# 17LiQi/MultimodalSignal

Hardware: AMD Instinct MI355X
Metric: train windows/sec (higher is better)
Workload: dtype f32; 1 GPU; CnnGruAttentionModel full train step (fwd+CE+bwd+Adam, dropout 0.5, BN batch stats), B=8192 windows/GPU x (6 ch, 3840 samples = 60 s @ 64 Hz), random-init weights; BASELINE.json configs[4] shape, the per-step work of configs[1]; batch_per_gpu=8192, channels=6, samples=3840, classes=2, parallelism=replica x1

## Files before the change

### multimodalsignal_amd/csrc/frontend.hip

```cpp
#include "msig_dev.h"

template <int CT, bool EO_ONLY = false>
__global__ __launch_bounds__(256) void gate_kernel(const float* __restrict__ x, const float* __restrict__ W1,
                                                   const float* __restrict__ W2, float* __restrict__ mean_out,
                                                   float* __restrict__ pre_out, float* __restrict__ s_out,
                                                   float* __restrict__ eo_out, int C, int T, int Cr, const FoldCtx fc) {
  FOLD_BEGIN; FS(x); FS(W1); FS(W2); FS(mean_out); FS(pre_out); FS(s_out); FS(eo_out);
  __shared__ float red[4][MSIG_MAX_C];
  __shared__ float red_eo[4][2 * MSIG_MAX_C];
  __shared__ float mean_s[MSIG_MAX_C];
  __shared__ float hid_s[MSIG_MAX_C / 4];
  const int b = blockIdx.x, tid = threadIdx.x, lane = tid & 63, w = tid >> 6;
  const float* xb = x + (size_t)b * C * T;
  if (CT > 0 && (T & 3) == 0) {
    constexpr int CN = CT > 0 ? CT : 1;
    float acc[CN], ev[CN], od[CN];
#pragma unroll
    for (int c = 0; c < CN; ++c) acc[c] = ev[c] = od[c] = 0.f;
    const int T4 = T / 4;
    constexpr int U = CN <= 4 ? 4 : 2;
    for (int i0 = tid; i0 < T4; i0 += 256 * U) {
      float4 q[U][CN];
#pragma unroll
      for (int u = 0; u < U; ++u) {
        const int i = i0 + 256 * u < T4 ? i0 + 256 * u : i0;
#pragma unroll
        for (int c = 0; c < CN; ++c) q[u][c] = ((const float4*)xb)[(size_t)c * T4 + i];
      }
#pragma unroll
      for (int u = 0; u < U; ++u)
        if (i0 + 256 * u < T4) {
#pragma unroll
          for (int c = 0; c < CN; ++c) {
            if (!EO_ONLY) acc[c] += (q[u][c].x + q[u][c].y) + (q[u][c].z + q[u][c].w);
            ev[c] += q[u][c].x + q[u][c].z; od[c] += q[u][c].y + q[u][c].w;
          }
        }
    }
#pragma unroll
    for (int c = 0; c < CN; ++c) {
      if (!EO_ONLY) {
        const float a = wave_sum(acc[c]);
        if (lane == 0) red[w][c] = a;
      }
      if (eo_out) {
        const float e = wave_sum(ev[c]), o = wave_sum(od[c]);
        if (lane == 0) { red_eo[w][2 * c] = e; red_eo[w][2 * c + 1] = o; }
      }
    }
  } else
  for (int c = 0; c < C; ++c) {
    const float* xc = xb + (size_t)c * T;
    float acc = 0.f, ev = 0.f, od = 0.f;
    if ((T & 3) == 0) {
      const float4* x4 = (const float4*)xc;
      for (int i = tid; i < T / 4; i += 256) {
        const float4 q = x4[i];
        if (!EO_ONLY) acc += (q.x + q.y) + (q.z + q.w);
        ev += q.x + q.z; od += q.y + q.w;
      }
    } else {
      for (int i = tid; i < T; i += 256) { const float v = xc[i]; if (!EO_ONLY) acc += v; if (i & 1) od += v; else ev += v; }
    }
    if (!EO_ONLY) {
      acc = wave_sum(acc);
      if (lane == 0) red[w][c] = acc;
    }
    if (eo_out) {
      ev = wave_sum(ev); od = wave_sum(od);
      if (lane == 0) { red_eo[w][2 * c] = ev; red_eo[w][2 * c + 1] = od; }
    }
  }
  __syncthreads();
  if (EO_ONLY) {
    if (tid < 2 * C) eo_out[(size_t)b * 2 * C + tid] = (red_eo[0][tid] + red_eo[1][tid]) + (red_eo[2][tid] + red_eo[3][tid]);
    return;
  }
  if (tid < C) {
    const float m = (red[0][tid] + red[1][tid] + red[2][tid] + red[3][tid]) / (float)T;
    mean_s[tid] = m;
    mean_out[(size_t)b * C + tid] = m;
  }
  if (eo_out && tid < 2 * C) eo_out[(size_t)b * 2 * C + tid] = (red_eo[0][tid] + red_eo[1][tid]) + (red_eo[2][tid] + red_eo[3][tid]);
  __syncthreads();
  if (tid < Cr) {
    float a = 0.f;
    for (int c = 0; c < C; ++c) a += W1[tid * C + c] * mean_s[c];
    pre_out[(size_t)b * Cr + tid] = a;
    hid_s[tid] = a > 0.f ? a : 0.f;
  }
  __syncthreads();
  if (tid < C) {
    float a = 0.f;
    for (int j = 0; j < Cr; ++j) a += W2[tid * Cr + j] * hid_s[j];
    s_out[(size_t)b * C + tid] = sigmoidf_fast(a);
  }
}

__global__ __launch_bounds__(256) void gate_scale_kernel(const float* __restrict__ x, const float* __restrict__ s, float* __restrict__ out,
                                                         int T, int64_t n_rows) {
  for (int64_t row = blockIdx.x; row < n_rows; row += gridDim.x) {
    const float sc = s[row];
    const float* xr = x + row * T;
    float* o = out + row * T;
    if ((T & 3) == 0 && (((uintptr_t)xr | (uintptr_t)o) & 15) == 0) {
      for (int i = threadIdx.x; i < T / 4; i += 256) {
        const float4 q = ((const float4*)xr)[i];
        ((float4*)o)[i] = make_float4(q.x * sc, q.y * sc, q.z * sc, q.w * sc);
      }
    } else {
      for (int i = threadIdx.x; i < T; i += 256) o[i] = xr[i] * sc;
    }
  }
}
int launch_channel_attention(const float* x, const float* W1, const float* W2, int B, int C, int T, float* out, float* s, float* scratch,
                             hipStream_t st) {
  const int Cr = C / 4;
  const FoldCtx fc = single_fold(nullptr);
  gate_kernel<0><<<dim3(B, 1, 1), 256, 0, st>>>(x, W1, W2, scratch, scratch + (size_t)B * C, s, nullptr, C, T, Cr, fc);
  MSIG_LAUNCH_CHECK();
  const int64_t rows = (int64_t)B * C;
  gate_scale_kernel<<<dim3((unsigned)(rows < 4096 ? rows : 4096)), 256, 0, st>>>(x, s, out, T, rows);
  MSIG_LAUNCH_CHECK();
  return 0;
}

#define C1_CHUNK 256
#define C1_XW (2 * C1_CHUNK + 8)
#define C1_XP (C1_XW / 2 + 4)
#define C1_MAXKM 28

template <bool DEINT>
__device__ __forceinline__ void stage_x_chunk(float* xs, const float* __restrict__ xb, int C, int T, int t0, int tid, int xstride = C1_XW) {
  const int g_base = 2 * t0 - 4;
  if ((T & 3) == 0) {
    for (int i = tid; i < C * (C1_XW / 4); i += 256) {
      const int c = i / (C1_XW / 4), i4 = i - c * (C1_XW / 4), g0 = g_base + 4 * i4;
      const int gc = g0 < 0 ? 0 : (g0 > T - 4 ? T - 4 : g0);
      float4 q = *(const float4*)(xb + (size_t)c * T + gc);
      if (g0 < 0 || g0 > T - 4) q = make_float4(0.f, 0.f, 0.f, 0.f);
      if (DEINT) {
        *(float2*)&xs[(2 * c) * C1_XP + 2 * i4] = make_float2(q.x, q.z);
        *(float2*)&xs[(2 * c + 1) * C1_XP + 2 * i4] = make_float2(q.y, q.w);
      } else {
        *(float4*)&xs[c * xstride + 4 * i4] = q;
      }
    }
  } else {
    for (int i = tid; i < C * C1_XW; i += 256) {
      const int c = i / C1_XW, j = i - c * C1_XW, g = g_base + j;
      const int gc = g < 0 ? 0 : (g > T - 1 ? T - 1 : g);
      float v = xb[(size_t)c * T + gc];
      if (g < 0 || g > T - 1 - (msig_negctl_length == 1 && t0 > 0 ? 1 : 0)) v = 0.f;
      if (DEINT) xs[(2 * c + (j & 1)) * C1_XP + (j >> 1)] = v; else xs[c * xstride + j] = v;
    }
  }
}

template <int CT, bool GATED = true>
__global__ __launch_bounds__(256) void conv1_fwd_kernel(const float* __restrict__ x, const float* __restrict__ w1,
                                                        const float* __restrict__ gate_s, float* __restrict__ y1,
                                                        float* __restrict__ part, int B, int Crt, int T, int L1,
                                                        int want_stats, const FoldCtx fc) {
  FOLD_BEGIN; FS(x); FS(w1); FS(gate_s); FS(y1); FS(part);
  extern __shared__ __attribute__((aligned(16))) float smem[];
  const int C = CT > 0 ? CT : Crt;
  const int K = C * 7, KM = (K + 3) / 4;
  constexpr int KMC = CT > 0 ? (CT * 7 + 3) / 4 : C1_MAXKM;
  float* xs = smem;
  float* ws = smem + 2 * C * C1_XP;
  const int tid = threadIdx.x, lane = tid & 63, w = tid >> 6, li = lane & 15, lq = lane >> 4;
  int xo[KMC];
#pragma unroll
  for (int m = 0; m < KMC; ++m) {
    const int k = 4 * m + lq, kc = k < K ? k : 0, c = kc / 7, kk = kc - 7 * c;
    xo[m] = (2 * c + ((kk + 1) & 1)) * C1_XP + ((kk + 1) >> 1);
  }
  const int nchunk = (L1 + C1_CHUNK - 1) / C1_CHUNK;
  const int nitems = B * nchunk;
  f32x4 ssum = {0.f, 0.f, 0.f, 0.f}, ssq = {0.f, 0.f, 0.f, 0.f};
  f32x4 dsum = {0.f, 0.f, 0.f, 0.f}, dsq = {0.f, 0.f, 0.f, 0.f}, piv = {0.f, 0.f, 0.f, 0.f};
  int nacc = 0;
  constexpr bool PIPE = CT > 0;
  constexpr int NX4 = PIPE ? (CT * (C1_XW / 4) + 255) / 256 : 1;
  constexpr int NWS = PIPE ? (4 * KMC * 16 + 255) / 256 : 1;
  const bool pipe = PIPE && (T & 3) == 0;
  float4 xr[NX4];
  float wfix[NWS], gr[NWS];
  if (GATED && pipe) {
#pragma unroll
    for (int j = 0; j < NWS; ++j) {
      const int i = tid + 256 * j, k = i >> 4, o = i & 15;
      wfix[j] = (i < 4 * KM * 16 && k < K) ? w1[o * K + k] : 0.f;
    }
  }
  auto prefetch = [&](int item) {
    const int b = item / nchunk, t0 = (item - b * nchunk) * C1_CHUNK, g_base = 2 * t0 - 4;
    const float* xb = x + (size_t)b * C * T;
#pragma unroll
    for (int j = 0; j < NX4; ++j) {
      const int i = tid + 256 * j, ic = i < C * (C1_XW / 4) ? i : 0;
      const int c = ic / (C1_XW / 4), i4 = ic - c * (C1_XW / 4), g0 = g_base + 4 * i4;
      const int gc = g0 < 0 ? 0 : (g0 > T - 4 ? T - 4 : g0);
      xr[j] = *(const float4*)(xb + (size_t)c * T + gc);
    }
    if (GATED) {
#pragma unroll
      for (int j = 0; j < NWS; ++j) {
        const int i = tid + 256 * j, k = i >> 4, kc = (i < 4 * KM * 16 && k < K) ? k : 0;
        gr[j] = gate_s[(size_t)b * C + kc / 7];
      }
    }
  };
  float wa[KMC];
  if (!GATED) {
#pragma unroll
    for (int m = 0; m < KMC; ++m) {
      const int k = 4 * m + lq;
      wa[m] = ((CT > 0 || m < KM) && k < K) ? w1[li * K + k] : 0.f;
    }
  }
  if (pipe && (int)blockIdx.x < nitems) prefetch(blockIdx.x);
  for (int item = blockIdx.x; item < nitems; item += gridDim.x) {
    const int b = item / nchunk, t0 = (item - b * nchunk) * C1_CHUNK;
    __syncthreads();
    if (pipe) {
      const int g_base = 2 * t0 - 4;
#pragma unroll
      for (int j = 0; j < NX4; ++j) {
        const int i = tid + 256 * j;
        if (i < C * (C1_XW / 4)) {
          const int c = i / (C1_XW / 4), i4 = i - c * (C1_XW / 4), g0 = g_base + 4 * i4;
          float4 q = xr[j];
          if (g0 < 0 || g0 > T - 4) q = make_float4(0.f, 0.f, 0.f, 0.f);
          *(float2*)&xs[(2 * c) * C1_XP + 2 * i4] = make_float2(q.x, q.z);
          *(float2*)&xs[(2 * c + 1) * C1_XP + 2 * i4] = make_float2(q.y, q.w);
        }
      }
      if (GATED) {
#pragma unroll
        for (int j = 0; j < NWS; ++j) {
          const int i = tid + 256 * j;
          if (i < 4 * KM * 16) ws[i] = wfix[j] * gr[j];
        }
      }
    } else {
      stage_x_chunk<true>(xs, x + (size_t)b * C * T, C, T, t0, tid);
      if (GATED) {
        for (int i = tid; i < 4 * KM * 16; i += 256) {
          const int k = i >> 4, o = i & 15, kc = k < K ? k : 0;
          const float v = w1[o * K + kc] * gate_s[(size_t)b * C + kc / 7];
          ws[i] = (k < K || (msig_negctl_range == 1 && CT == 0)) ? v : 0.f;
        }
      }
    }
    __syncthreads();
    if (pipe && item + (int)gridDim.x < nitems) prefetch(item + gridDim.x);
    if (GATED) {
#pragma unroll
      for (int m = 0; m < KMC; ++m) wa[m] = (CT > 0 || m < KM) ? ws[(4 * m + lq) * 16 + li] : 0.f;
    }
#pragma unroll
    for (int pbi = 0; pbi < 4; ++pbi) {
      const int pl = (w * 4 + pbi) * 16 + li;
      f32x4 acc0 = {0.f, 0.f, 0.f, 0.f}, acc1 = {0.f, 0.f, 0.f, 0.f};
#pragma unroll
      for (int m = 0; m < KMC; m += 2) {
        if (CT > 0 || m < KM) acc0 = mfma16(wa[m], xs[xo[m] + pl], acc0);
        if (m + 1 < KMC && (CT > 0 || m + 1 < KM)) acc1 = mfma16(wa[m + 1], xs[xo[m + 1] + pl], acc1);
      }
      const f32x4 acc = acc0 + acc1;
      const int t = t0 + pl;
      if (t < L1) {
        *(float4*)(y1 + ((size_t)b * L1 + t) * 16 + lq * 4) = make_float4(acc[0], acc[1], acc[2], acc[3]);
#pragma unroll
        for (int e = 0; e < 4; ++e) { ssum[e] += acc[e]; ssq[e] += acc[e] * acc[e]; }
        if (nacc == 0) piv = acc;
        ++nacc;
#pragma unroll
        for (int e = 0; e < 4; ++e) { const float dv = acc[e] - piv[e]; dsum[e] += dv; dsq[e] += dv * dv; }
      }
    }
  }
  if (want_stats) {
    __syncthreads();
    float* red = smem;
#pragma unroll
    for (int e = 0; e < 4; ++e) {
      float s1 = ssum[e], s2 = ssq[e];
#pragma unroll
      for (int o = 8; o > 0; o >>= 1) { s1 += __shfl_xor(s1, o, 64); s2 += __shfl_xor(s2, o, 64); }
      if (li == 0) { red[w * 32 + lq * 4 + e] = s1; red[w * 32 + 16 + lq * 4 + e] = s2; }
    }
    __syncthreads();
    if (tid < 32) part[(size_t)blockIdx.x * 32 + tid] = red[tid] + red[32 + tid] + red[64 + tid] + red[96 + tid];
    double* redd = (double*)(smem + 4 * 32);
#pragma unroll
    for (int e = 0; e < 4; ++e) {
      double s1, s2;
      bn_unshift(nacc, piv[e], dsum[e], dsq[e], s1, s2);
#pragma unroll
      for (int o = 8; o > 0; o >>= 1) { s1 += __shfl_xor(s1, o, 64); s2 += __shfl_xor(s2, o, 64); }
      if (li == 0) { redd[w * 32 + lq * 4 + e] = s1; redd[w * 32 + 16 + lq * 4 + e] = s2; }
    }
    __syncthreads();
    if (tid < 32) bn_shifted_part(part, 16)[(size_t)blockIdx.x * 32 + tid] = (redd[tid] + redd[32 + tid]) + (redd[64 + tid] + redd[96 + tid]);
  }
}

#define C2_CHUNK 128
#define C2_ROWS (2 * C2_CHUNK + 3)
#define C2_PS 20
#define PC_YROWS (2 * C2_ROWS + 1)
__device__ __forceinline__ int first_argmax3(float l, float c, float r);
__global__ __launch_bounds__(256, 2) void pool1_conv2_fwd_kernel(const float* __restrict__ y1, const float* __restrict__ stat1,
                                                                 float* __restrict__ p1, uint8_t* __restrict__ code1,
                                                                 const float* __restrict__ w2, float* __restrict__ y2,
                                                                 float* __restrict__ part, int B, int L1, int P1, int L2,
                                                                 int want_stats, const FoldCtx fc) {
  FOLD_BEGIN; FS(y1); FS(stat1); FS(p1); FS(code1); FS(w2); FS(y2); FS(part);
  __shared__ __attribute__((aligned(16))) float zs[PC_YROWS * C2_PS];
  __shared__ __attribute__((aligned(16))) float ps[C2_ROWS * C2_PS];
  __shared__ float red[4 * 64];
  const int tid = threadIdx.x, lane = tid & 63, w = tid >> 6, li = lane & 15, lq = lane >> 4;
  float A[2][20];
#pragma unroll
  for (int ob = 0; ob < 2; ++ob)
#pragma unroll
    for (int m = 0; m < 20; ++m) A[ob][m] = w2[((ob * 16 + li) * 16 + lq * 4 + (m & 3)) * 5 + (m >> 2)];
  const int nchunk = (L2 + C2_CHUNK - 1) / C2_CHUNK;
  const int nitems = B * nchunk;
  f32x4 ssum[2] = {{0.f, 0.f, 0.f, 0.f}, {0.f, 0.f, 0.f, 0.f}}, ssq[2] = {{0.f, 0.f, 0.f, 0.f}, {0.f, 0.f, 0.f, 0.f}};
  f32x4 dsum[2] = {{0.f, 0.f, 0.f, 0.f}, {0.f, 0.f, 0.f, 0.f}}, dsq[2] = {{0.f, 0.f, 0.f, 0.f}, {0.f, 0.f, 0.f, 0.f}};
  f32x4 piv[2] = {{0.f, 0.f, 0.f, 0.f}, {0.f, 0.f, 0.f, 0.f}};
  int nacc = 0;
  const float NINF = -__builtin_huge_valf();
  const int c4s = tid & 3;
  const float4 sc4 = *(const float4*)(stat1 + 2 * 16 + c4s * 4), sh4 = *(const float4*)(stat1 + 3 * 16 + c4s * 4);
  const float scv[4] = {sc4.x, sc4.y, sc4.z, sc4.w}, shv[4] = {sh4.x, sh4.y, sh4.z, sh4.w};
  constexpr int NY4 = (PC_YROWS * 4 + 255) / 256, NP4 = (C2_ROWS * 4 + 255) / 256;
  float4 yr[NY4];
  auto prefetch = [&](int item) {
    const int b = item / nchunk, t0 = (item - b * nchunk) * C2_CHUNK, ty0 = 4 * t0 - 5;
#pragma unroll
    for (int j = 0; j < NY4; ++j) {
      const int i = tid + 256 * j, row = i >> 2, ty = ty0 + row;
      const int tc = ty < 0 ? 0 : (ty > L1 - 1 ? L1 - 1 : ty);
      yr[j] = *(const float4*)(y1 + ((size_t)b * L1 + tc) * 16 + c4s * 4);
    }
  };
  if ((int)blockIdx.x < nitems) prefetch(blockIdx.x);
  for (int item = blockIdx.x; item < nitems; item += gridDim.x) {
    const int b = item / nchunk, t0 = (item - b * nchunk) * C2_CHUNK;
    const int base = 2 * t0 - 2, ty0 = 4 * t0 - 5;
    __syncthreads();
#pragma unroll
    for (int j = 0; j < NY4; ++j) {
      const int i = tid + 256 * j, row = i >> 2, ty = ty0 + row;
      if (i < PC_YROWS * 4) {
        const bool ok = ty >= 0 && ty < L1;
        const float qv[4] = {yr[j].x, yr[j].y, yr[j].z, yr[j].w};
        float z[4];
#pragma unroll
        for (int e = 0; e < 4; ++e) z[e] = ok ? qv[e] * scv[e] + shv[e] : NINF;
        *(float4*)&zs[row * C2_PS + c4s * 4] = make_float4(z[0], z[1], z[2], z[3]);
      }
    }
    __syncthreads();
    if (item + (int)gridDim.x < nitems) prefetch(item + gridDim.x);
#pragma unroll
    for (int j = 0; j < NP4; ++j) {
      const int i = tid + 256 * j, row = i >> 2, pp = base + row;
      if (i < C2_ROWS * 4) {
        float best[4] = {0.f, 0.f, 0.f, 0.f};
        if (pp >= 0 && pp < P1) {
          const float4 l4 = *(const float4*)&zs[(2 * row) * C2_PS + c4s * 4], m4 = *(const float4*)&zs[(2 * row + 1) * C2_PS + c4s * 4],
                       r4 = *(const float4*)&zs[(2 * row + 2) * C2_PS + c4s * 4];
          const float zl[4] = {l4.x, l4.y, l4.z, l4.w}, zc[4] = {m4.x, m4.y, m4.z, m4.w}, zr[4] = {r4.x, r4.y, r4.z, r4.w};
          unsigned cd = 0;
#pragma unroll
          for (int e = 0; e < 4; ++e) {
            const int win = first_argmax3(zl[e], zc[e], zr[e]);
            const float m = win == 0 ? zl[e] : (win == 1 ? zc[e] : zr[e]);
            best[e] = fmaxf(m, 0.f);
            cd |= (unsigned)(m > 0.f ? win : 3) << (2 * e);
          }
          if (row >= 2 && row < 2 + 2 * C2_CHUNK) {
            *(float4*)(p1 + ((size_t)b * P1 + pp) * 16 + c4s * 4) = make_float4(best[0], best[1], best[2], best[3]);
            if (code1) code1[((size_t)b * P1 + pp) * 4 + c4s] = (uint8_t)cd;
          }
        }
        *(float4*)&ps[row * C2_PS + c4s * 4] = make_float4(best[0], best[1], best[2], best[3]);
      }
    }
    __syncthreads();
#pragma unroll
    for (int pbi = 0; pbi < 2; ++pbi) {
      const int pl = (w * 2 + pbi) * 16 + li;
      f32x4 acc0 = {0.f, 0.f, 0.f, 0.f}, acc1 = {0.f, 0.f, 0.f, 0.f};
#pragma unroll
      for (int kk = 0; kk < 5; ++kk) {
        const float4 q = *(const float4*)&ps[(2 * pl + kk) * C2_PS + lq * 4];
        acc0 = mfma16(A[0][4 * kk + 0], q.x, acc0); acc1 = mfma16(A[1][4 * kk + 0], q.x, acc1);
        acc0 = mfma16(A[0][4 * kk + 1], q.y, acc0); acc1 = mfma16(A[1][4 * kk + 1], q.y, acc1);
        acc0 = mfma16(A[0][4 * kk + 2], q.z, acc0); acc1 = mfma16(A[1][4 * kk + 2], q.z, acc1);
        acc0 = mfma16(A[0][4 * kk + 3], q.w, acc0); acc1 = mfma16(A[1][4 * kk + 3], q.w, acc1);
      }
      const int t = t0 + pl;
      if (t < L2) {
        float* dst = y2 + ((size_t)b * L2 + t) * 32 + lq * 4;
        *(float4*)dst = make_float4(acc0[0], acc0[1], acc0[2], acc0[3]);
        *(float4*)(dst + 16) = make_float4(acc1[0], acc1[1], acc1[2], acc1[3]);
#pragma unroll
        for (int e = 0; e < 4; ++e) {
          ssum[0][e] += acc0[e]; ssq[0][e] += acc0[e] * acc0[e];
          ssum[1][e] += acc1[e]; ssq[1][e] += acc1[e] * acc1[e];
        }
        if (nacc == 0) { piv[0] = acc0; piv[1] = acc1; }
        ++nacc;
#pragma unroll
        for (int e = 0; e < 4; ++e) {
          const float d0 = acc0[e] - piv[0][e], d1 = acc1[e] - piv[1][e];
          dsum[0][e] += d0; dsq[0][e] += d0 * d0;
          dsum[1][e] += d1; dsq[1][e] += d1 * d1;
        }
      }
    }
  }
  if (want_stats) {
#pragma unroll
    for (int ob = 0; ob < 2; ++ob)
#pragma unroll
      for (int e = 0; e < 4; ++e) {
        float s1 = ssum[ob][e], s2 = ssq[ob][e];
#pragma unroll
        for (int o = 8; o > 0; o >>= 1) { s1 += __shfl_xor(s1, o, 64); s2 += __shfl_xor(s2, o, 64); }
        if (li == 0) { red[w * 64 + ob * 16 + lq * 4 + e] = s1; red[w * 64 + 32 + ob * 16 + lq * 4 + e] = s2; }
      }
    __syncthreads();
    if (tid < 64) part[(size_t)blockIdx.x * 64 + tid] = red[tid] + red[64 + tid] + red[128 + tid] + red[192 + tid];
    double* redd = (double*)zs;
#pragma unroll
    for (int ob = 0; ob < 2; ++ob)
#pragma unroll
      for (int e = 0; e < 4; ++e) {
        double s1, s2;
        bn_unshift(nacc, piv[ob][e], dsum[ob][e], dsq[ob][e], s1, s2);
#pragma unroll
        for (int o = 8; o > 0; o >>= 1) { s1 += __shfl_xor(s1, o, 64); s2 += __shfl_xor(s2, o, 64); }
        if (li == 0) { redd[w * 64 + ob * 16 + lq * 4 + e] = s1; redd[w * 64 + 32 + ob * 16 + lq * 4 + e] = s2; }
      }
    __syncthreads();
    if (tid < 64) bn_shifted_part(part, 32)[(size_t)blockIdx.x * 64 + tid] = (redd[tid] + redd[64 + tid]) + (redd[128 + tid] + redd[192 + tid]);
  }
}


__global__ __launch_bounds__(FIN_THREADS) void bn_finalize_kernel(const float* __restrict__ part, int nrows, int CH, double count,
                                                          const float* __restrict__ gamma, const float* __restrict__ beta,
                                                          float* __restrict__ run_mean, float* __restrict__ run_var,
                                                          int64_t* __restrict__ nbt, float momentum, float eps,
                                                          int training, float* __restrict__ stat, const FoldCtx fc) {
  FOLD_BEGIN; FS(part); FS(gamma); FS(beta); FS(run_mean); FS(run_var); FS(nbt); FS(stat);
  __shared__ double red[FIN_THREADS];
  const int tid = threadIdx.x;
  if (training) {
    double s1, s2;
    const bool shifted = bn_batch_sums(part, nrows, CH, count, red, s1, s2);
    if (tid < CH) {
      const double mean = s1 / count;
      double var = s2 / count - mean * mean;
      if (var < 0.0) var = 0.0;
      const float invstd = (float)(msig_negctl_input == 2 ? 1.0 / (sqrt(var) + (double)eps) : 1.0 / sqrt(var + (double)eps));
      const float sc = (msig_negctl_regime == 3 ? fabsf(gamma[tid]) : gamma[tid]) * invstd;
      stat[tid] = (float)mean;
      stat[CH + tid] = invstd;
      stat[2 * CH + tid] = sc;
      stat[3 * CH + tid] = beta[tid] - (float)mean * sc;
      stat[4 * CH + tid] = shifted ? (float)((mean - (double)(float)mean) * (double)invstd) : 0.f;
      const double unbiased = count > 1.0 ? var * count / (count - 1.0) : var;
      float new_mean, new_var;
      bn_running_update(momentum, (float)mean, (float)unbiased, run_mean[tid], run_var[tid], new_mean, new_var);
      run_mean[tid] = new_mean;
      run_var[tid] = new_var;
    }
    if (tid == 0) nbt[0] += 1;
  } else if (tid < CH) {
    const float invstd = 1.0f / sqrtf(run_var[tid] + eps);
    const float sc = (msig_negctl_regime == 3 ? fabsf(gamma[tid]) : gamma[tid]) * invstd;
    stat[tid] = run_mean[tid];
    stat[CH + tid] = invstd;
    stat[2 * CH + tid] = sc;
    stat[3 * CH + tid] = beta[tid] - run_mean[tid] * sc;
    stat[4 * CH + tid] = 0.f;
  }
}

__device__ __forceinline__ int first_argmax3(float l, float c, float r) {
  int a = 0; float m = l;
  if (c > m) { a = 1; m = c; }
  if (r > m) { a = 2; }
  return a;
}

template <int CH>
__global__ __launch_bounds__(256) void bn_relu_pool_kernel(const float* __restrict__ y, const float* __restrict__ stat,
                                                           float* __restrict__ p, uint8_t* __restrict__ code, int B, int L, int P,
                                                           const FoldCtx fc) {
  FOLD_BEGIN; FS(y); FS(stat); FS(p); FS(code);
  constexpr int C4 = CH / 4;
  const int64_t total = (int64_t)B * P * C4;
  const float NINF = -__builtin_huge_valf();
  for (int64_t i = (int64_t)blockIdx.x * 256 + threadIdx.x; i < total; i += (int64_t)gridDim.x * 256) {
    const int c4 = (int)(i % C4);
    const int64_t bp = i / C4;
    const int pp = (int)(bp % P), b = (int)(bp / P);
    const float4 sc = *(const float4*)(stat + 2 * CH + c4 * 4), sh = *(const float4*)(stat + 3 * CH + c4 * 4);
    const float scv[4] = {sc.x, sc.y, sc.z, sc.w}, shv[4] = {sh.x, sh.y, sh.z, sh.w};
    float z[3][4];
#pragma unroll
    for (int j = 0; j < 3; ++j) {
      const int t = 2 * pp - 1 + j;
      const bool ok = t >= 0 && t < L;
      const float4 q = *(const float4*)(y + ((size_t)b * L + (ok ? t : 2 * pp)) * CH + c4 * 4);
      const float qv[4] = {q.x, q.y, q.z, q.w};
#pragma unroll
      for (int e = 0; e < 4; ++e) z[j][e] = ok ? qv[e] * scv[e] + shv[e] : NINF;
    }
    float best[4];
    unsigned cd = 0;
#pragma unroll
    for (int e = 0; e < 4; ++e) {
      const int win = first_argmax3(z[0][e], z[1][e], z[2][e]);
      const float m = win == 0 ? z[0][e] : (win == 1 ? z[1][e] : z[2][e]);
      best[e] = fmaxf(m, 0.f);
      cd |= (unsigned)(m > 0.f ? win : 3) << (2 * e);
    }
    *(float4*)(p + ((size_t)b * P + pp) * CH + c4 * 4) = make_float4(best[0], best[1], best[2], best[3]);
    if (code) code[((size_t)b * P + pp) * C4 + c4] = (uint8_t)cd;
  }
}

struct RoutedRaw { float4 g0, g1; unsigned c0, c1; };
template <int CH>
__device__ __forceinline__ RoutedRaw routed_load(const float* __restrict__ dp, const uint8_t* __restrict__ code, int b, int t, int P, int c4) {
  constexpr int C4 = CH / 4;
  const int ph = t >> 1, ph1 = (ph + 1 < P) ? ph + 1 : ph;
  RoutedRaw r;
  r.g0 = *(const float4*)(dp + ((size_t)b * P + ph) * CH + c4 * 4);
  r.g1 = *(const float4*)(dp + ((size_t)b * P + ph1) * CH + c4 * 4);
  r.c0 = code[((size_t)b * P + ph) * C4 + c4];
  r.c1 = code[((size_t)b * P + ph1) * C4 + c4];
  return r;
}
__device__ __forceinline__ float4 routed_dz(const RoutedRaw& r, int t, int P) {
  const bool odd = t & 1, has1 = odd && ((t >> 1) + 1 < P);
  const unsigned want0 = odd ? 2u : 1u;
  const float g0[4] = {r.g0.x, r.g0.y, r.g0.z, r.g0.w}, g1[4] = {r.g1.x, r.g1.y, r.g1.z, r.g1.w};
  float o[4];
#pragma unroll
  for (int e = 0; e < 4; ++e) {
    o[e] = (((r.c0 >> (2 * e)) & 3u) == want0) ? g0[e] : 0.f;
    if (has1 && ((r.c1 >> (2 * e)) & 3u) == 0u) o[e] += g1[e];
  }
  return make_float4(o[0], o[1], o[2], o[3]);
}

template <int CH>
__global__ __launch_bounds__(256) void pool_bn_bwd_pass1(const float* __restrict__ dp_a, const float* __restrict__ dp_b,
                                                         const uint8_t* __restrict__ code, const float* __restrict__ y,
                                                         const float* __restrict__ stat, float* __restrict__ dz,
                                                         float* __restrict__ part, int B, int L, int P, const FoldCtx fc) {
  FOLD_BEGIN; FS(dp_a); FS(dp_b); FS(code); FS(y); FS(stat); FS(dz); FS(part);
  constexpr int C4 = CH / 4;
  __shared__ float red[256 * 8];
  const int c4 = threadIdx.x % C4;
  float s1[4] = {0.f, 0.f, 0.f, 0.f}, s2[4] = {0.f, 0.f, 0.f, 0.f};
  float mean[4], invstd[4];
#pragma unroll
  for (int e = 0; e < 4; ++e) { mean[e] = stat[c4 * 4 + e]; invstd[e] = stat[CH + c4 * 4 + e]; }
  const int64_t total = (int64_t)B * L * C4;
  for (int64_t i = (int64_t)blockIdx.x * 256 + threadIdx.x; i < total; i += (int64_t)gridDim.x * 256) {
    const int64_t bt = i / C4;
    const int t = (int)(bt % L), b = (int)(bt / L);
    RoutedRaw r = routed_load<CH>(dp_a, code, b, t, P, c4);
    if (dp_b) {
      const RoutedRaw r2 = routed_load<CH>(dp_b, code, b, t, P, c4);
      r.g0.x += r2.g0.x; r.g0.y += r2.g0.y; r.g0.z += r2.g0.z; r.g0.w += r2.g0.w;
      r.g1.x += r2.g1.x; r.g1.y += r2.g1.y; r.g1.z += r2.g1.z; r.g1.w += r2.g1.w;
    }
    const float4 d = routed_dz(r, t, P);
    const float4 yq = *(const float4*)(y + ((size_t)b * L + t) * CH + c4 * 4);
    *(float4*)(dz + ((size_t)b * L + t) * CH + c4 * 4) = d;
    const float dv[4] = {d.x, d.y, d.z, d.w}, yv[4] = {yq.x, yq.y, yq.z, yq.w};
#pragma unroll
    for (int e = 0; e < 4; ++e) { s1[e] += dv[e]; s2[e] += dv[e] * (yv[e] - mean[e]) * invstd[e]; }
  }
#pragma unroll
  for (int e = 0; e < 4; ++e) { red[threadIdx.x * 8 + e] = s1[e]; red[threadIdx.x * 8 + 4 + e] = s2[e]; }
  __syncthreads();
  if (threadIdx.x < 2 * CH) {
    const int which = threadIdx.x / CH, ch = threadIdx.x % CH, cc4 = ch / 4, e = ch % 4;
    float acc = 0.f;
    for (int t = cc4; t < 256; t += C4) acc += red[t * 8 + which * 4 + e];
    part[(size_t)blockIdx.x * 2 * CH + threadIdx.x] = acc;
  }
}

__global__ __launch_bounds__(FIN_THREADS) void bn_bwd_finalize_kernel(const float* __restrict__ part, int nrows, int CH, double count,
                                                              const float* __restrict__ stat, float* __restrict__ cstat,
                                                              float* __restrict__ dgamma, float* __restrict__ dbeta, int batch_stats,
                                                              const FoldCtx fc) {
  FOLD_BEGIN; FS(part); FS(stat); FS(cstat); FS(dgamma); FS(dbeta);
  __shared__ double red[FIN_THREADS];
  const int tid = threadIdx.x, ncol = 2 * CH;
  fin_colsums(part, nrows, ncol, red);
  if (tid < ncol) {
    const int ch = tid < CH ? tid : tid - CH;
    const double sdz = red[ch], m = batch_stats ? (double)stat[4 * CH + ch] : 0.0;
    const double g = red[CH + ch] - m * sdz;
    const double s = tid < CH ? sdz - m * g : g;
    if (tid < CH) dbeta[tid] = (float)sdz; else dgamma[ch] = (float)g;
    cstat[tid] = batch_stats ? (float)(s / count) : 0.f;
  }
}

#define D2_UCH 128
#define D2_ROWS (D2_UCH + 2)
#define D2_PS 36
#define W2_PROWS (2 * D2_UCH + 3)

__global__ __launch_bounds__(256) void conv2_bwd_kernel(const float* __restrict__ dz2, const float* __restrict__ y2,
                                                        const float* __restrict__ stat, const float* __restrict__ cstat,
                                                        const float* __restrict__ w2, const float* __restrict__ p1,
                                                        float* __restrict__ dp1, float* __restrict__ part, int B, int P1, int L2,
                                                        const FoldCtx fc) {
  FOLD_BEGIN; FS(dz2); FS(y2); FS(stat); FS(cstat); FS(w2); FS(p1); FS(dp1); FS(part);
  __shared__ __attribute__((aligned(16))) float ds_[D2_ROWS * D2_PS];
  __shared__ __attribute__((aligned(16))) float ps[W2_PROWS * C2_PS];
  const int tid = threadIdx.x, lane = tid & 63, w = tid >> 6, li = lane & 15, lq = lane >> 4;
  float Ae[24], Ao[16];
#pragma unroll
  for (int m = 0; m < 24; ++m) Ae[m] = w2[((lq * 8 + (m & 7)) * 16 + li) * 5 + 2 * (m >> 3)];
#pragma unroll
  for (int m = 0; m < 16; ++m) Ao[m] = w2[((lq * 8 + (m & 7)) * 16 + li) * 5 + 1 + 2 * (m >> 3)];
  f32x4 acc[2][5];
#pragma unroll
  for (int ob = 0; ob < 2; ++ob)
#pragma unroll
    for (int kk = 0; kk < 5; ++kk) acc[ob][kk] = (f32x4){0.f, 0.f, 0.f, 0.f};
  const int nchunk = (L2 + D2_UCH - 1) / D2_UCH;
  const int nitems = B * nchunk;
  float bn_mean[4], bn_inv[4], bn_sc[4], bn_c1[4], bn_c2[4];
#pragma unroll
  for (int e = 0; e < 4; ++e) {
    const int ch = (tid & 7) * 4 + e;
    bn_mean[e] = stat[ch]; bn_inv[e] = stat[32 + ch]; bn_sc[e] = stat[64 + ch]; bn_c1[e] = cstat[ch]; bn_c2[e] = cstat[32 + ch];
  }
  constexpr int ND4 = (D2_ROWS * 8 + 255) / 256, NP4 = (W2_PROWS * 4 + 255) / 256;
  float4 dr[ND4], yr[ND4], qr[NP4];
  auto prefetch = [&](int item) {
    const int b = item / nchunk, t0 = (item - b * nchunk) * D2_UCH, base = 2 * t0 - 2;
#pragma unroll
    for (int j = 0; j < ND4; ++j) {
      const int i = tid + 256 * j, row = i >> 3, c4 = i & 7, t = t0 - 1 + row;
      const int tc = t < 0 ? 0 : (t > L2 - 1 ? L2 - 1 : t);
      dr[j] = *(const float4*)(dz2 + ((size_t)b * L2 + tc) * 32 + c4 * 4);
      yr[j] = *(const float4*)(y2 + ((size_t)b * L2 + tc) * 32 + c4 * 4);
    }
#pragma unroll
    for (int j = 0; j < NP4; ++j) {
      const int i = tid + 256 * j, row = i >> 2, c4 = i & 3, src = base + row;
      const int sc = src < 0 ? 0 : (src > P1 - 1 ? P1 - 1 : src);
      qr[j] = *(const float4*)(p1 + ((size_t)b * P1 + sc) * 16 + c4 * 4);
    }
  };
  if ((int)blockIdx.x < nitems) prefetch(blockIdx.x);
  for (int item = blockIdx.x; item < nitems; item += gridDim.x) {
    const int b = item / nchunk, t0 = (item - b * nchunk) * D2_UCH;
    __syncthreads();
#pragma unroll
    for (int j = 0; j < ND4; ++j) {
      const int i = tid + 256 * j, row = i >> 3, c4 = i & 7, t = t0 - 1 + row;
      if (i < D2_ROWS * 8) {
        const float4 dzv = dr[j];
        float4 q;
        q.x = bn_sc[0] * (dzv.x - bn_c1[0] - (yr[j].x - bn_mean[0]) * bn_inv[0] * bn_c2[0]);
        q.y = bn_sc[1] * (dzv.y - bn_c1[1] - (yr[j].y - bn_mean[1]) * bn_inv[1] * bn_c2[1]);
        q.z = bn_sc[2] * (dzv.z - bn_c1[2] - (yr[j].z - bn_mean[2]) * bn_inv[2] * bn_c2[2]);
        q.w = bn_sc[3] * (dzv.w - bn_c1[3] - (yr[j].w - bn_mean[3]) * bn_inv[3] * bn_c2[3]);
        if (t < 0 || t >= L2) q = make_float4(0.f, 0.f, 0.f, 0.f);
        *(float4*)&ds_[row * D2_PS + c4 * 4] = q;
      }
    }
    const int base = 2 * t0 - 2;
#pragma unroll
    for (int j = 0; j < NP4; ++j) {
      const int i = tid + 256 * j, row = i >> 2, c4 = i & 3, src = base + row;
      if (i < W2_PROWS * 4) {
        float4 q = qr[j];
        if (src < 0 || src >= P1) q = make_float4(0.f, 0.f, 0.f, 0.f);
        *(float4*)&ps[row * C2_PS + c4 * 4] = q;
      }
    }
    __syncthreads();
    if (item + (int)gridDim.x < nitems) prefetch(item + gridDim.x);
#pragma unroll
    for (int ubi = 0; ubi < 2; ++ubi) {
      const int ul = (w * 2 + ubi) * 16 + li;
      f32x4 ae0 = {0.f, 0.f, 0.f, 0.f}, ae1 = {0.f, 0.f, 0.f, 0.f}, ao0 = {0.f, 0.f, 0.f, 0.f}, ao1 = {0.f, 0.f, 0.f, 0.f};
#pragma unroll
      for (int ti = 0; ti < 3; ++ti) {
        const float* rowp = &ds_[(ul + 2 - ti) * D2_PS + lq * 8];
        const float4 q0 = *(const float4*)rowp, q1 = *(const float4*)(rowp + 4);
        const float qv[8] = {q0.x, q0.y, q0.z, q0.w, q1.x, q1.y, q1.z, q1.w};
#pragma unroll
        for (int mm = 0; mm < 8; ++mm) {
          if (mm & 1) ae1 = mfma16(Ae[ti * 8 + mm], qv[mm], ae1); else ae0 = mfma16(Ae[ti * 8 + mm], qv[mm], ae0);
          if (ti < 2) { if (mm & 1) ao1 = mfma16(Ao[ti * 8 + mm], qv[mm], ao1); else ao0 = mfma16(Ao[ti * 8 + mm], qv[mm], ao0); }
        }
      }
      const int u = t0 + ul;
      if (2 * u < P1)
        *(float4*)(dp1 + ((size_t)b * P1 + 2 * u) * 16 + lq * 4) = make_float4(ae0[0] + ae1[0], ae0[1] + ae1[1], ae0[2] + ae1[2], ae0[3] + ae1[3]);
      if (2 * u + 1 < P1)
        *(float4*)(dp1 + ((size_t)b * P1 + 2 * u + 1) * 16 + lq * 4) = make_float4(ao0[0] + ao1[0], ao0[1] + ao1[1], ao0[2] + ao1[2], ao0[3] + ao1[3]);
    }
#pragma unroll 2
    for (int m = 0; m < D2_UCH / 16; ++m) {
      const int tl = w * 32 + 4 * m + lq;
      const float a0 = ds_[(tl + 1) * D2_PS + li], a1 = ds_[(tl + 1) * D2_PS + 16 + li];
#pragma unroll
      for (int kk = 0; kk < 5; ++kk) {
        const float bv = ps[(2 * tl + kk) * C2_PS + li];
        acc[0][kk] = mfma16(a0, bv, acc[0][kk]);
        acc[1][kk] = mfma16(a1, bv, acc[1][kk]);
      }
    }
  }
  __syncthreads();
  float* red = ds_;
  for (int ww = 0; ww < 4; ++ww) {
    if (w == ww) {
#pragma unroll
// ... 589 lines not shown
```

Baseline: 1.052 million windows/s.

## Stream conv1 activations into LDS via direct global-to-LDS DMA in pool1_conv2

Replaces the register-prefetch plus BN-transform-store stage in pool1_conv2_fwd_kernel with global_load_lds_dwordx4 DMA that writes raw y1 rows straight into LDS in an even/odd de-interleaved layout. The BN affine and the bounds masking move into the maxpool step, which removes one LDS write pass, one barrier and the register staging. The pooled buffer gets an XOR-swizzled layout to avoid bank conflicts in the MFMA reads. The inline-asm m0 handling and the hand-counted vmcnt waits are fragile, and interleaving with the p1/code1 stores could miscount outstanding ops.

```diff
diff --git a/multimodalsignal_amd/csrc/frontend.hip b/multimodalsignal_amd/csrc/frontend.hip
--- a/multimodalsignal_amd/csrc/frontend.hip
+++ b/multimodalsignal_amd/csrc/frontend.hip
@@ -1,4 +1,5 @@
 #include "msig_dev.h"
+#include "lds_dma.h"
 
 template <int CT, bool EO_ONLY = false>
 __global__ __launch_bounds__(256) void gate_kernel(const float* __restrict__ x, const float* __restrict__ W1,
@@ -312,15 +313,20 @@
 #define C2_ROWS (2 * C2_CHUNK + 3)
 #define C2_PS 20
 #define PC_YROWS (2 * C2_ROWS + 1)
+#define PC_EROWS (C2_ROWS + 1)
+#define PC_PIECES ((PC_YROWS * 4 + 63) / 64)
+#define PC_NDJ ((PC_PIECES + 3) / 4)
 __device__ __forceinline__ int first_argmax3(float l, float c, float r);
+__device__ __forceinline__ int pc_prow(int R, int c4) { return (R ^ ((R >> 3) & 1)) * 16 + ((c4 ^ ((R >> 1) & 3)) << 2); }
+#define PC_LDS_PAD 4096
 __global__ __launch_bounds__(256, 2) void pool1_conv2_fwd_kernel(const float* __restrict__ y1, const float* __restrict__ stat1,
                                                                  float* __restrict__ p1, uint8_t* __restrict__ code1,
                                                                  const float* __restrict__ w2, float* __restrict__ y2,
                                                                  float* __restrict__ part, int B, int L1, int P1, int L2,
                                                                  int want_stats, const FoldCtx fc) {
   FOLD_BEGIN; FS(y1); FS(stat1); FS(p1); FS(code1); FS(w2); FS(y2); FS(part);
-  __shared__ __attribute__((aligned(16))) float zs[PC_YROWS * C2_PS];
-  __shared__ __attribute__((aligned(16))) float ps[C2_ROWS * C2_PS];
+  __shared__ __attribute__((aligned(16))) float raw[PC_PIECES * 256 + PC_LDS_PAD];
+  __shared__ __attribute__((aligned(16))) float ps[PC_EROWS * 16];
   __shared__ float red[4 * 64];
   const int tid = threadIdx.x, lane = tid & 63, w = tid >> 6, li = lane & 15, lq = lane >> 4;
   float A[2][20];
@@ -338,50 +344,50 @@
   const int c4s = tid & 3;
   const float4 sc4 = *(const float4*)(stat1 + 2 * 16 + c4s * 4), sh4 = *(const float4*)(stat1 + 3 * 16 + c4s * 4);
   const float scv[4] = {sc4.x, sc4.y, sc4.z, sc4.w}, shv[4] = {sh4.x, sh4.y, sh4.z, sh4.w};
-  constexpr int NY4 = (PC_YROWS * 4 + 255) / 256, NP4 = (C2_ROWS * 4 + 255) / 256;
-  float4 yr[NY4];
-  auto prefetch = [&](int item) {
-    const int b = item / nchunk, t0 = (item - b * nchunk) * C2_CHUNK, ty0 = 4 * t0 - 5;
-#pragma unroll
-    for (int j = 0; j < NY4; ++j) {
-      const int i = tid + 256 * j, row = i >> 2, ty = ty0 + row;
-      const int tc = ty < 0 ? 0 : (ty > L1 - 1 ? L1 - 1 : ty);
-      yr[j] = *(const float4*)(y1 + ((size_t)b * L1 + tc) * 16 + c4s * 4);
-    }
+  constexpr int NP4 = (C2_ROWS * 4 + 255) / 256;
+  int drow[PC_NDJ];
+#pragma unroll
+  for (int j = 0; j < PC_NDJ; ++j) {
+    const int rl = ((w + 4 * j) * 64 + lane) >> 2;
+    drow[j] = rl < PC_EROWS ? 2 * rl : (rl < PC_YROWS ? 2 * (rl - PC_EROWS) + 1 : PC_YROWS - 1);
+  }
+  const int wu = __builtin_amdgcn_readfirstlane(w);
+  const uint32_t raw_dst = lds_dma_addr(raw) + wu * 1024;
+  auto issue = [&](int item) {
+    const int b = item / nchunk, ty0 = 4 * (item - b * nchunk) * C2_CHUNK - 5;
+    const char* src = lds_dma_uniform(y1 + (size_t)b * L1 * 16);
+#pragma unroll
+    for (int j = 0; j < PC_NDJ; ++j)
+      if (wu + 4 * j < PC_PIECES) {
+        const int ty = ty0 + drow[j];
+        const int tc = ty < 0 ? 0 : (ty > L1 - 1 ? L1 - 1 : ty);
+        lds_dma16((uint32_t)(tc * 16 + c4s * 4) * 4u, src, raw_dst + 4096 * j);
+      }
   };
-  if ((int)blockIdx.x < nitems) prefetch(blockIdx.x);
+  if ((int)blockIdx.x < nitems) issue(blockIdx.x);
+  bool stores4 = false;
   for (int item = blockIdx.x; item < nitems; item += gridDim.x) {
     const int b = item / nchunk, t0 = (item - b * nchunk) * C2_CHUNK;
     const int base = 2 * t0 - 2, ty0 = 4 * t0 - 5;
-    __syncthreads();
-#pragma unroll
-    for (int j = 0; j < NY4; ++j) {
-      const int i = tid + 256 * j, row = i >> 2, ty = ty0 + row;
-      if (i < PC_YROWS * 4) {
-        const bool ok = ty >= 0 && ty < L1;
-        const float qv[4] = {yr[j].x, yr[j].y, yr[j].z, yr[j].w};
-        float z[4];
-#pragma unroll
-        for (int e = 0; e < 4; ++e) z[e] = ok ? qv[e] * scv[e] + shv[e] : NINF;
-        *(float4*)&zs[row * C2_PS + c4s * 4] = make_float4(z[0], z[1], z[2], z[3]);
-      }
-    }
-    __syncthreads();
-    if (item + (int)gridDim.x < nitems) prefetch(item + gridDim.x);
+    if (stores4) LDS_DMA_WAIT(4); else LDS_DMA_WAIT(0);
+    __syncthreads();
 #pragma unroll
     for (int j = 0; j < NP4; ++j) {
       const int i = tid + 256 * j, row = i >> 2, pp = base + row;
       if (i < C2_ROWS * 4) {
         float best[4] = {0.f, 0.f, 0.f, 0.f};
         if (pp >= 0 && pp < P1) {
-          const float4 l4 = *(const float4*)&zs[(2 * row) * C2_PS + c4s * 4], m4 = *(const float4*)&zs[(2 * row + 1) * C2_PS + c4s * 4],
-                       r4 = *(const float4*)&zs[(2 * row + 2) * C2_PS + c4s * 4];
-          const float zl[4] = {l4.x, l4.y, l4.z, l4.w}, zc[4] = {m4.x, m4.y, m4.z, m4.w}, zr[4] = {r4.x, r4.y, r4.z, r4.w};
+          const int tyl = ty0 + 2 * row;
+          const bool okl = tyl >= 0 && tyl < L1, okc = tyl + 1 >= 0 && tyl + 1 < L1, okr = tyl + 2 >= 0 && tyl + 2 < L1;
+          const float4 l4 = *(const float4*)&raw[4 * i], m4 = *(const float4*)&raw[PC_EROWS * 16 + 4 * i], r4 = *(const float4*)&raw[16 + 4 * i];
+          const float ql[4] = {l4.x, l4.y, l4.z, l4.w}, qc[4] = {m4.x, m4.y, m4.z, m4.w}, qr[4] = {r4.x, r4.y, r4.z, r4.w};
           unsigned cd = 0;
 #pragma unroll
           for (int e = 0; e < 4; ++e) {
-            const int win = first_argmax3(zl[e], zc[e], zr[e]);
-            const float m = win == 0 ? zl[e] : (win == 1 ? zc[e] : zr[e]);
+            const float zl = okl ? ql[e] * scv[e] + shv[e] : NINF, zc = okc ? qc[e] * scv[e] + shv[e] : NINF,
+                        zr = okr ? qr[e] * scv[e] + shv[e] : NINF;
+            const int win = first_argmax3(zl, zc, zr);
+            const float m = win == 0 ? zl : (win == 1 ? zc : zr);
             best[e] = fmaxf(m, 0.f);
             cd |= (unsigned)(m > 0.f ? win : 3) << (2 * e);
           }
@@ -390,17 +396,19 @@
             if (code1) code1[((size_t)b * P1 + pp) * 4 + c4s] = (uint8_t)cd;
           }
         }
-        *(float4*)&ps[row * C2_PS + c4s * 4] = make_float4(best[0], best[1], best[2], best[3]);
-      }
-    }
-    __syncthreads();
+        *(float4*)&ps[pc_prow(row, c4s)] = make_float4(best[0], best[1], best[2], best[3]);
+      }
+    }
+    __syncthreads();
+    if (item + (int)gridDim.x < nitems) issue(item + gridDim.x);
+    stores4 = t0 + C2_CHUNK <= L2;
 #pragma unroll
     for (int pbi = 0; pbi < 2; ++pbi) {
       const int pl = (w * 2 + pbi) * 16 + li;
       f32x4 acc0 = {0.f, 0.f, 0.f, 0.f}, acc1 = {0.f, 0.f, 0.f, 0.f};
 #pragma unroll
       for (int kk = 0; kk < 5; ++kk) {
-        const float4 q = *(const float4*)&ps[(2 * pl + kk) * C2_PS + lq * 4];
+        const float4 q = *(const float4*)&ps[pc_prow(2 * pl + kk, lq)];
         acc0 = mfma16(A[0][4 * kk + 0], q.x, acc0); acc1 = mfma16(A[1][4 * kk + 0], q.x, acc1);
         acc0 = mfma16(A[0][4 * kk + 1], q.y, acc0); acc1 = mfma16(A[1][4 * kk + 1], q.y, acc1);
         acc0 = mfma16(A[0][4 * kk + 2], q.z, acc0); acc1 = mfma16(A[1][4 * kk + 2], q.z, acc1);
@@ -439,7 +447,7 @@
       }
     __syncthreads();
     if (tid < 64) part[(size_t)blockIdx.x * 64 + tid] = red[tid] + red[64 + tid] + red[128 + tid] + red[192 + tid];
-    double* redd = (double*)zs;
+    double* redd = (double*)raw;
 #pragma unroll
     for (int ob = 0; ob < 2; ++ob)
 #pragma unroll
diff --git a/multimodalsignal_amd/csrc/lds_dma.h b/multimodalsignal_amd/csrc/lds_dma.h
--- /dev/null
+++ b/multimodalsignal_amd/csrc/lds_dma.h
@@ -0,0 +1,17 @@
+#pragma once
+#include <hip/hip_runtime.h>
+#include <stdint.h>
+
+#define LDS_DMA_WAIT(n) asm volatile("s_waitcnt vmcnt(%0)" :: "n"(n) : "memory")
+
+__device__ __forceinline__ const char* lds_dma_uniform(const void* p) {
+  const uint64_t v = (uint64_t)(uintptr_t)p;
+  const uint32_t lo = __builtin_amdgcn_readfirstlane((uint32_t)v), hi = __builtin_amdgcn_readfirstlane((uint32_t)(v >> 32));
+  return (const char*)(uintptr_t)(((uint64_t)hi << 32) | lo);
+}
+__device__ __forceinline__ uint32_t lds_dma_addr(const void* lds) { return __builtin_amdgcn_readfirstlane((uint32_t)(uintptr_t)lds); }
+__device__ __forceinline__ void lds_dma16(uint32_t voff, const char* sbase, uint32_t lds_dst) {
+  uint32_t keep;
+  asm volatile("s_mov_b32 %0, m0\n\ts_mov_b32 m0, %3\n\ts_nop 0\n\tglobal_load_lds_dwordx4 %1, %2\n\ts_mov_b32 m0, %0"
+               : "=&s"(keep) : "v"(voff), "s"(sbase), "s"(lds_dst) : "memory");
+}
```

Measured after the change: 1.061 million windows/s, median of 6. Within noise of the previous version (+0.9%).
